# will-rowe/groot

Hardware: AMD Instinct MI355X
Metric: Mreads/s aligned (higher is better)
Workload: dtype u64

## Files before the change

### groot_amd/csrc/hip/align.hip

```cpp
#include <hip/hip_runtime.h>

#include "kernels_align.hpp"
#include "kernels_lean.hpp"
#include "launch.hpp"

namespace groot {

void launch_align(uint32_t pw, const AlignArgs &a, dim3 grid, hipStream_t st)
{
    const size_t lds = a.lds_stride_dw ? (size_t)kBlock * a.lds_stride_dw * 4 + 16 : 0;
    if (pw == 3) {
        if (lds) hipLaunchKernelGGL((align_kernel<3, true>), grid, dim3(kBlock), lds, st, a);
        else hipLaunchKernelGGL((align_kernel<3, false>), grid, dim3(kBlock), 0, st, a);
    } else if (pw == 11) {
        if (lds) hipLaunchKernelGGL((align_kernel<11, true>), grid, dim3(kBlock), lds, st, a);
        else hipLaunchKernelGGL((align_kernel<11, false>), grid, dim3(kBlock), 0, st, a);
    }
}

void launch_align_lean(uint32_t pw, const LeanArgs &a, dim3 grid, hipStream_t st)
{
    if (pw != 3) return;
    const size_t lds = (size_t)kBlock * a.lds_stride_dw * 4;
    if (a.max_len <= 128) hipLaunchKernelGGL((align_lean_kernel<3, 4>), grid, dim3(kBlock), lds, st, a);
    else if (a.max_len <= 160) hipLaunchKernelGGL((align_lean_kernel<3, 5>), grid, dim3(kBlock), lds, st, a);
    else hipLaunchKernelGGL((align_lean_kernel<3, 8>), grid, dim3(kBlock), lds, st, a);
}

void launch_align_path(uint32_t pw, const LeanArgs &a, dim3 grid, hipStream_t st)
{
    if (pw != 3) return;
// ... 8 lines not shown
```

### groot_amd/csrc/hip/ctx.hpp

```cpp
#pragma once

#include <hip/hip_runtime.h>

#include <algorithm>
#include <array>
#include <atomic>
#include <cstdlib>
#include <deque>
#include <map>
#include <memory>
#include <string>
#include <thread>
#include <vector>

#include "device_types.hpp"

using namespace groot;


template <class T> struct DevBuf {
    T *p = nullptr;
    size_t n = 0;
    hipError_t alloc(size_t count)
    {
// ... 24 lines not shown
    hipError_t reserve(size_t count) { return count <= n && p ? hipSuccess : alloc(count); }
    void release()
    {
        if (p) (void)hipHostFree(p);
        p = nullptr;
        n = 0;
    }
    ~PinBuf() { release(); }
};

struct Knobs {
    bool no_outcome_table = false, no_text_table = false, no_sig = false, force_rccl = false, small_buffers = false, open_stats = false, poison = false, lean = false, no_path = false,
         shared_slow = false, serial_tail = false, assign_global = false;
    uint32_t ec_slots = 0;
    uint32_t acov_slots = 0;
    static Knobs read()
    {
        Knobs k;
        k.no_outcome_table = getenv("GROOT_NO_OUTCOME_TABLE") != nullptr; k.no_text_table = getenv("GROOT_NO_TEXT_TABLE") != nullptr;
        k.no_sig = getenv("GROOT_NO_SIG") != nullptr;                     k.force_rccl = getenv("GROOT_FORCE_RCCL") != nullptr;
        k.small_buffers = getenv("GROOT_TEST_SMALL_BUFFERS") != nullptr;  k.open_stats = getenv("GROOT_OPEN_STATS") != nullptr;
        k.poison = getenv("GROOT_TEST_POISON") != nullptr;
        k.lean = getenv("GROOT_LEAN") != nullptr;
        k.no_path = getenv("GROOT_NO_PATH_PASS") != nullptr;
        k.shared_slow = getenv("GROOT_TEST_SHARED_SLOW") != nullptr;
        k.serial_tail = getenv("GROOT_SERIAL_TAIL") != nullptr;
        k.assign_global = getenv("GROOT_TEST_ASSIGN_GLOBAL") != nullptr;
        if (const char *e = getenv("GROOT_TEST_EC_SLOTS")) k.ec_slots = (uint32_t)std::min<unsigned long>(strtoul(e, nullptr, 10), 1ul << 30);
        if (const char *e = getenv("GROOT_TEST_ACOV_SLOTS")) k.acov_slots = (uint32_t)std::min<unsigned long>(strtoul(e, nullptr, 10), 1ul << 30);
        return k;
    }
};

namespace groot {
struct EcTable;
struct AcovTable;
}

struct EcBufs {
    uint32_t cap = 0;
    DevBuf<uint32_t> claim, graph;
    DevBuf<uint64_t> mask;
    DevBuf<unsigned long long> cnt;
    DevBuf<uint32_t> serial;
// ... 114 lines not shown
    hipEvent_t ev_seed = nullptr;
    hipEvent_t ev_walk = nullptr;
    hipEvent_t ev_h2d0 = nullptr, ev_h2d = nullptr, ev_compute = nullptr, ev_ctr = nullptr, ev_d2h0 = nullptr, ev_d2h = nullptr;
    hipEvent_t ev[14]{};
    groot_counts counts{};
    int status = GROOT_OK;
    std::string status_msg;
    groot_stage_ms ms{};
    SlotCounters ct;
    const uint8_t *seq() const { return input == IN_DEVICE ? ext_seq : d_seq.p; }
    const uint64_t *off() const { return input == IN_DEVICE ? ext_off : d_off.p; }
};

struct WorkSet {
    DevBuf<uint32_t> seed_count, seed_win, perm, perm_count, trav_cnt, tab_idx;
    DevBuf<uint32_t> perm2;
    DevBuf<uint4> packed;
    DevBuf<ReadRec> read_rec;
    DevBuf<uint4> vitem, split_list;
    DevBuf<uint32_t> vcount;
    DevBuf<groot_trav> trav_first;
    DevBuf<uint64_t> mask_first, sketches;
    DevBuf<groot_trav> ovf_trav;
    DevBuf<uint64_t> ovf_mask;
    DevBuf<uint32_t> ovf_cnt;
    hipEvent_t ev_free = nullptr;
    bool used = false;
    Slot *owner = nullptr;
    uint64_t ticket = 0;
};

// ... 131 lines not shown
```

### groot_amd/csrc/hip/device_types.hpp

```cpp
#pragma once

#include <cstdint>

#include <hip/hip_runtime.h>

#include "groot_hip.h"

namespace groot {

constexpr int kBlock = 256;
constexpr uint32_t kEmpty = 0xFFFFFFFFu;

enum : uint32_t {
    kFlagShortRead = 1u,
    kFlagLongRead = 2u,
    kFlagSeedOverflow = 4u,
    kFlagTravOverflow = 8u,
    kFlagOrdOverflow = 16u,
    kFlagOvfOverflow = 32u,
    kFlagQOverflow = 64u,
};

constexpr uint32_t kIncrCap = 8;
constexpr uint32_t kIncrCapBig = 2048;
constexpr uint32_t kSeedShards = 64, kSeedShardStride = 16;
constexpr uint32_t kOvfShards = 256;
// ... 182 lines not shown
    groot_trav *ovf_trav;
    uint64_t *ovf_mask;
    uint32_t *ovf_cnt;
    uint32_t ovf_cap;
    uint64_t *stk_hdr;
    uint64_t *stk_mask;
    uint32_t n_threads, stk_depth;
    uint32_t lds_stride_dw;
    uint32_t *incr_cnt, *incr_win;
    uint32_t incr_cap;
    uint32_t head_lanes;
    uint32_t round_lanes;
    const uint4 *vitem;
    const uint32_t *vcount;
    uint32_t vcap;
    const uint32_t *n_perm;
    const uint32_t *rest;
    uint32_t rest_lo;
    uint32_t refill;
    DeviceCounters *ctr;
};

struct alignas(16) LeanNode {
    uint32_t seq_off;
    uint32_t seq_len;
    uint32_t deg_kids;
    uint32_t pad;
    uint32_t edges[4];
    uint64_t first32;
    uint64_t mask[3];
};
static_assert(sizeof(LeanNode) == 64, "lean node record is one 64-byte line");
constexpr uint32_t kLeanNo = 0x80000000u;
// ... 14 lines not shown
    const WinRec *win_rec;
    const uint32_t *q_row;
    const uint8_t *seq;
    const uint4 *packed;
    uint32_t packed_q;
    const uint32_t *perm;
    const ReadRec *read_rec;
    uint32_t n_reads, first_read_id, n_windows, k;
    uint32_t update_weights;
    uint32_t lds_stride_dw;
    uint32_t max_len;
    uint32_t *attempts;
    groot_trav *trav_first;
    uint64_t *mask_first;
    uint32_t *trav_cnt;
    uint32_t *left;
    uint32_t *left_cnt;
    uint4 *stk;
    groot_trav *ovf_trav;
    uint64_t *ovf_mask;
    uint32_t *ovf_cnt;
    uint32_t ovf_cap;
    DeviceCounters *ctr;
    const uint4 *path_node;
    const uint32_t *path_text;
    const uint32_t *path_tag;
    const uint32_t *path_nodes;
    const uint64_t *path_tab;
    uint4 *hold;
};

// ... 4 lines not shown
```

### groot_amd/csrc/hip/groot_hip.hip

```cpp
#include <cstring>

#include <hip/hip_runtime.h>
#include <rocprim/rocprim.hpp>

#include <dlfcn.h>

#include <algorithm>
#include <cmath>
#include <cstdarg>
#include <cstdio>
#include <atomic>
#include <chrono>
#include <deque>
#include <iterator>
#include <array>
#include <map>
#include <tuple>
#include <memory>
#include <numeric>
#include <string>
#include <thread>
#include <vector>

#include "../common/cpus.hpp"
#include "../common/view_check.hpp"
#include "counters.hpp"
#include "ctx.hpp"
#include "kernels_misc.hpp"
#include "kernels_path.hpp"
#include "launch.hpp"

using namespace groot;

__attribute__((constructor)) static void groot_hw_queues() { setenv("GPU_MAX_HW_QUEUES", "8", 0); }

static thread_local std::string g_open_err;

static thread_local bool tl_background = false;

namespace groot {

int fail(groot_ctx *ctx, int code, const char *fmt, ...)
{
    char buf[1024];
    va_list ap;
// ... 434 lines not shown
    a.attempts = c->attempts_ptr;
    a.node_rec = c->node_rec.p;
    a.trav_first = w->trav_first.p;
    a.mask_first = w->mask_first.p;
    a.trav_cnt = w->trav_cnt.p;
    a.ovf_trav = w->ovf_trav.p;
    a.ovf_mask = w->ovf_mask.p;
    a.ovf_cnt = w->ovf_cnt.p;
    a.ovf_cap = c->ovf_cap;
    if (c->vcap) { a.vitem = w->vitem.p; a.vcount = w->vcount.p; a.vcap = c->vcap; }
    a.stk_hdr = c->stk_hdr.p;
    a.stk_mask = c->stk_mask.p;
    uint32_t blocks = std::min<uint32_t>((s->n_reads + kBlock - 1) / kBlock, c->align_threads / kBlock);
    if (c->dfs_frac < kSparseBelow && c->dfs_frac * (double)s->n_reads < 16.0 * (double)(blocks * (kBlock / 64))) blocks = std::max(1u, blocks / 2);
    else if (error_batch(c, s) && blocks >= 4) blocks /= 2;
    if ((s->lean_used || s->path_used) && c->lean_left_frac < 0.25) {
        uint32_t want = (uint32_t)(c->lean_left_frac * 1.25 * (double)s->n_reads / 64.0 / (kBlock / 64)) + 1u;
        blocks = std::max(1u, std::min(blocks, std::max(want, c->n_cu)));
    }
    a.n_threads = blocks * kBlock;
    a.stk_depth = c->stk_depth;
    {
        const uint32_t stride = (2 + 4 * ((s->max_len + 27) / 16)) | 1u;
        a.lds_stride_dw = (size_t)kBlock * stride * 4 <= 64 * 1024 ? stride : 0;
    }
    if (c->tab_capture) {
        a.incr_cnt = c->incr_cnt.p; a.incr_win = c->incr_win.p; a.incr_cap = c->incr_cap;
        HIP_TRY(c, hipMemsetAsync(c->incr_cnt.p, 0, (size_t)s->n_reads * sizeof(uint32_t), c->tstream));
    }
    a.head_lanes = s->mixed_len ? 16u : 0u;
#ifndef GROOT_REFILL_ERR
#define GROOT_REFILL_ERR 48
#endif
#ifndef GROOT_REFILL_MIXED
#define GROOT_REFILL_MIXED 2
#endif
    a.refill = s->mixed_len ? (uint32_t)GROOT_REFILL_MIXED : (error_batch(c, s) ? (uint32_t)GROOT_REFILL_ERR : 64u);
#ifdef GROOT_WORK_COUNTERS
    if (const char *e = getenv("GROOT_DEV_ROUND")) a.round_lanes = (uint32_t)atoi(e);
#endif
    a.ctr = s->d_ctr.p;
    const bool first_pass = s->lean_used || s->path_used;
    hipStream_t walk = first_pass ? c->astream : c->tstream;
    HIP_TRY(c, hipMemsetAsync(w->ovf_cnt.p, 0, (kOvfShards + 3) * sizeof(uint32_t), walk));
    const uint32_t lean_stride = lean_stride_dw(s->max_len);
    if (first_pass) {
        LeanArgs l{};
        l.nodes = c->lean_nodes.p; l.ext = c->lean_ext.p; l.bases2 = c->bases2.p; l.cn_pre2 = c->cn_pre2.p; l.win_ok = c->win_ok.p;
        l.win_rec = c->dix.win_rec; l.node_l2b = c->dix.node_l2b; l.q_row = c->q_row.p;
        l.seq = s->seq(); l.packed = s->packed_q ? w->packed.p : nullptr; l.packed_q = s->packed_q; l.perm = w->perm.p; l.read_rec = w->read_rec.p;
        l.n_reads = s->n_reads; l.first_read_id = s->first_read_id; l.n_windows = c->n_windows; l.k = c->k;
        l.update_weights = update_weights ? 1 : 0;
        l.lds_stride_dw = lean_stride; l.max_len = s->max_len;
        l.attempts = c->attempts_ptr;
        l.trav_first = w->trav_first.p; l.mask_first = w->mask_first.p; l.trav_cnt = w->trav_cnt.p;
        l.left = w->perm2.p; l.left_cnt = w->ovf_cnt.p + kOvfShards + 2; l.ctr = s->d_ctr.p;
        l.stk = c->lean_stk.p; l.ovf_trav = w->ovf_trav.p; l.ovf_mask = w->ovf_mask.p; l.ovf_cnt = w->ovf_cnt.p; l.ovf_cap = c->ovf_cap;
        const uint32_t lean_blocks = std::min<uint32_t>((s->n_reads + kBlock - 1) / kBlock, (uint32_t)(c->dfs_frac * 1.05 * (double)s->n_reads / kBlock) + 64u);
        if (s->path_used) {
            l.path_node = c->path_node.p; l.path_text = c->path_text.p; l.path_tag = c->path_tag.p; l.path_nodes = c->path_nodes.p; l.path_tab = c->path_tab.p;
            l.hold = c->path_hold.p;
            launch_align_path(c->pw, l, dim3(lean_blocks), c->astream);
        } else launch_align_lean(c->pw, l, dim3(lean_blocks), c->astream);
        HIP_TRY(c, hipGetLastError());
        a.perm = w->perm2.p;
        a.n_perm = l.left_cnt;
        a.rest = w->perm.p;
        a.rest_lo = lean_blocks * (uint32_t)kBlock;
        if (c->profiling) HIP_TRY(c, hipEventRecord(s->ev[13], c->astream));
        if (c->tstream != c->astream) {
            HIP_TRY(c, hipEventRecord(s->ev_walk, c->astream));
            HIP_TRY(c, hipStreamWaitEvent(c->tstream, s->ev_walk, 0));
        }
    }
    launch_align(c->pw, a, dim3(blocks), c->tstream);
    HIP_TRY(c, hipGetLastError());
    return GROOT_OK;
}

static int launch_order_stage(groot_ctx *c, Slot *s, bool update_weights)
{
    WorkSet *w = &c->ws[s->set];
    const uint32_t n = s->n_reads;
// ... 47 lines not shown


static int run_batch_async(groot_ctx *c, Slot *s, bool update_weights)
{
    WorkSet *w = &c->ws[s->set];
    if (w->used) HIP_TRY(c, hipStreamWaitEvent(c->stream, w->ev_free, 0));
    HIP_TRY(c, hipMemsetAsync(s->d_ctr.p, 0, sizeof(DeviceCounters), c->stream));
    if (c->kn.poison) {
        const size_t n = s->n_reads;
        HIP_TRY(c, hipMemsetAsync(w->seed_count.p, 0, n * sizeof(uint32_t), c->stream));
        HIP_TRY(c, hipMemsetAsync(w->read_rec.p, 0, n * sizeof(ReadRec), c->stream));
        HIP_TRY(c, hipMemsetAsync(w->trav_cnt.p, 0, n * sizeof(uint32_t), c->stream));
        HIP_TRY(c, hipMemsetAsync(c->sort_key.p, 0xFF, n * sizeof(uint32_t), c->stream));
        if (w->tab_idx.p) HIP_TRY(c, hipMemsetAsync(w->tab_idx.p, 0xFF, n * sizeof(uint32_t), c->stream));
        HIP_TRY(c, hipMemsetAsync(c->todo_list.p, 0, n * sizeof(uint32_t), c->stream));
    }
    if (c->profiling) HIP_TRY(c, hipEventRecord(s->ev[1], c->stream));
    if (int rc = launch_seed_stage(c, s, update_weights)) return rc;
    if (c->profiling) HIP_TRY(c, hipEventRecord(s->ev[3], c->stream));
    HIP_TRY(c, hipEventRecord(s->ev_seed, c->stream));
    s->lean_used = c->lean && !c->tab_capture && s->n_reads && s->max_len <= kLeanMaxLen && c->dfs_frac >= 0.02;
    s->path_used = c->path && !c->tab_capture && s->n_reads && s->max_len <= kLeanMaxLen && c->dfs_frac >= 0.02;
    hipStream_t start = s->lean_used || s->path_used ? c->astream : c->tstream;
    HIP_TRY(c, hipStreamWaitEvent(start, s->ev_seed, 0));
    if (c->profiling) HIP_TRY(c, hipEventRecord(s->ev[11], start));
    if (int rc = launch_align_stage(c, s, update_weights)) return rc;
    if (c->profiling) HIP_TRY(c, hipEventRecord(s->ev[4], c->tstream));
    if (int rc = launch_order_stage(c, s, update_weights)) return rc;
    if (c->profiling) HIP_TRY(c, hipEventRecord(s->ev[5], c->tstream));
    HIP_TRY(c, hipEventRecord(w->ev_free, c->tstream));
// ... 432 lines not shown
}

}

extern "C" {

void groot_params_default(groot_params *p)
{
    if (!p) return;
    memset(p, 0, sizeof *p);
    p->containment_threshold = 0.99;
    p->max_read_len = 256;
    p->max_batch_reads = 1u << 20;
    p->max_seeds_per_read = 8;
    p->pipeline_depth = 3;
}

int groot_hip_device_count(int *n)
{
    if (!n) return GROOT_E_INVALID;
    int c = 0;
    hipError_t e = hipGetDeviceCount(&c);
    if (e != hipSuccess) {
        *n = 0;
        return fail(nullptr, GROOT_E_DEVICE, "hipGetDeviceCount: %s", hipGetErrorString(e));
    }
    *n = c;
    return GROOT_OK;
}

// ... 1069 lines not shown
    HIP_TRY(c, c->long_count.alloc(4));
    HIP_TRY(c, hipMemset(c->long_count.p, 0, 4 * sizeof(uint32_t)));
    {
        std::vector<uint32_t> iota(R);
        std::iota(iota.begin(), iota.end(), 0u);
        HIP_TRY(c, upload(c->perm_in, iota.data(), iota.size()));
    }
    if (int rc = alloc_seed_slots(c, c->prm.max_seeds_per_read)) return rc;
    c->vcap = c->kn.small_buffers ? 8u : std::max<uint32_t>(4096, R / 4);
    for (WorkSet &w : c->ws) {
        HIP_TRY(c, w.seed_count.alloc(R));
        HIP_TRY(c, w.read_rec.alloc(R));
        HIP_TRY(c, w.perm.alloc(R));
        HIP_TRY(c, w.perm_count.alloc(4));
        if (c->lean || c->path) {
            HIP_TRY(c, w.perm2.alloc(R));
            HIP_TRY(c, w.packed.alloc((size_t)R * (c->prm.max_read_len <= 128 ? 2 : 4)));
        }
        if (c->prm.keep_sketches) HIP_TRY(c, w.sketches.alloc((size_t)R * s));
        HIP_TRY(c, w.trav_first.alloc((size_t)R + c->vcap));
        HIP_TRY(c, w.mask_first.alloc(((size_t)R + c->vcap) * c->pw));
        HIP_TRY(c, w.trav_cnt.alloc((size_t)R + c->vcap));
        HIP_TRY(c, w.vitem.alloc(std::max<uint32_t>(c->vcap, 1)));
        HIP_TRY(c, w.split_list.alloc(kLongListCap));
        HIP_TRY(c, w.vcount.alloc(4));
        HIP_TRY(c, hipMemset(w.vcount.p, 0, 4 * sizeof(uint32_t)));
    }
    HIP_TRY(c, c->trav_off.alloc(R));
    if (c->lean || c->path) HIP_TRY(c, c->lean_stk.alloc((size_t)R * 4));
    if (c->path) HIP_TRY(c, c->path_hold.alloc((size_t)R * 3 * kPathHold));
    for (WorkSet &w : c->ws) HIP_TRY(c, w.ovf_cnt.alloc(kOvfShards + 3));
// ... 828 lines not shown
```

### groot_amd/csrc/hip/kernels_align.hpp

```cpp
#pragma once

#include "kernels_common.hpp"

namespace groot {


enum : uint32_t { PH_FETCH, PH_SCAN, PH_DFS, PH_WAIT, PH_DONE, PH_FORK, PH_FORKWAIT, PH_JOIN };
#ifndef GROOT_FORK_MIN
#define GROOT_FORK_MIN 3
#endif
constexpr uint32_t kForkMin = GROOT_FORK_MIN;
constexpr uint32_t kClsHelper = 0x1000u;
constexpr uint32_t kCoopMin = 6;
constexpr uint32_t kCoopWant = 0xFFFFFFFEu;
#ifndef GROOT_COOP_MAX_ASK
#define GROOT_COOP_MAX_ASK 8
#endif
constexpr uint32_t kCoopMaxAsk = GROOT_COOP_MAX_ASK;
#ifndef GROOT_TL_LATE_US
#define GROOT_TL_LATE_US 3000
#endif
#ifndef GROOT_WAVE_CHUNK
#define GROOT_WAVE_CHUNK 128
#endif
constexpr uint32_t kWaveChunk = GROOT_WAVE_CHUNK;

__device__ __forceinline__ uint64_t match_or_n(uint64_t x, unsigned c)
{
    return ~(nonzero_bytes(x ^ (kOnes * c)) & nonzero_bytes(x ^ (kOnes * 'N'))) & kHi1;
}
__device__ __forceinline__ uint64_t low_bytes(int n) { return n <= 0 ? 0 : (n >= 8 ? kHi1 : (kHi1 >> (8 * (8 - n)))); }

template <int PW> struct RecRegs {
    static constexpr int NQ = (int)(sizeof(NodeRec<PW>) / 16);
    uint32_t d[NQ * 4];
    __device__ __forceinline__ void load(const NodeRec<PW> *rp)
    {
        const uint4 *q = reinterpret_cast<const uint4 *>(rp);
#pragma unroll
        for (int i = 0; i < NQ; i++) {
            const uint4 v = q[i];
            d[4 * i] = v.x; d[4 * i + 1] = v.y; d[4 * i + 2] = v.z; d[4 * i + 3] = v.w;
        }
#pragma unroll
        for (int i = 0; i < NQ * 4; i++) asm volatile("" : "+v"(d[i]));
    }
// ... 26 lines not shown
#endif
    unsigned long long alns = 0, mapped = 0, multimapped = 0, panics = 0;
#ifdef GROOT_WORK_COUNTERS
    uint32_t ev = 0;
    uint32_t wc_iter = 0, wc_round0 = 0;
    unsigned long long wc_t[3] = {0, 0, 0};
    uint32_t wc_n[3] = {0, 0, 0};
    uint32_t wc_n0[3] = {0, 0, 0};
#define GROOT_EV(i) (ev |= 1u << (i))
#else
#define GROOT_EV(i) ((void)0)
#endif

    uint32_t phase = PH_WAIT;
    const uint32_t nv = a.vitem ? min((uint32_t)__builtin_amdgcn_readfirstlane((int)*a.vcount), a.vcap) : 0u;
    const uint32_t n_seeded = min(a.n_reads, (uint32_t)__builtin_amdgcn_readfirstlane((int)a.ctr->seeded_reads));
    const uint32_t n_list = a.n_perm ? min(a.n_reads, (uint32_t)__builtin_amdgcn_readfirstlane((int)*a.n_perm)) : n_seeded;
    const uint32_t n_rest = a.rest && n_seeded > a.rest_lo ? n_seeded - a.rest_lo : 0u;
    const uint32_t n_todo = nv + (a.perm ? min(a.n_reads, n_list + n_rest) : a.n_reads);
#ifndef GROOT_MIXED_ROUND_LANES
#define GROOT_MIXED_ROUND_LANES 32
#endif
    uint32_t U = a.head_lanes ? (uint32_t)GROOT_MIXED_ROUND_LANES : 64u;
    if (a.round_lanes) U = a.round_lanes;
    else
        while (U > 1u && n_todo < U * (gridDim.x * (uint32_t)(kBlock / 64))) U >>= 1;
    const uint32_t n_rounds = (n_todo + U - 1u) / U;
    const uint32_t head_rounds = (n_rounds >> 3) | 1u;
    const uint32_t Uh = a.head_lanes ? min(a.head_lanes, U) : U;
    const uint32_t head_slots = min(head_rounds * U, n_todo);
    const uint32_t head_small = (head_slots + Uh - 1u) / Uh;
    uint32_t chunk_len = 0, chunk_base = 0;
    bool head_done = head_small == 0;
    const uint32_t chunk_rounds = a.head_lanes ? 1u : kWaveChunk / 64u;
    auto take_chunk = [&]() {
        uint32_t c = 0, tail = 0;
        if ((threadIdx.x & 63) == 0) {
            if (!head_done) c = atomicAdd(a.ovf_cnt + kOvfShards, 1u);
            if (head_done || c >= head_small) {
                tail = 1;
                c = atomicAdd(a.ovf_cnt + kOvfShards + 1, chunk_rounds);
            }
        }
        c = (uint32_t)__builtin_amdgcn_readfirstlane((int)c);
        tail = (uint32_t)__builtin_amdgcn_readfirstlane((int)tail);
        if (tail) {
            head_done = true;
            const unsigned long long b = (unsigned long long)head_slots + (unsigned long long)c * U;
            chunk_base = b > 0xFFFFFFFFull ? 0xFFFFFFFFu : (uint32_t)b;
            chunk_len = chunk_rounds * U;
        } else {
            chunk_base = c * Uh;
            chunk_len = min(Uh, head_slots - chunk_base);
        }
    };
    take_chunk();
#if defined(GROOT_WORK_COUNTERS) && GROOT_WORK_COUNTERS == 3
    const unsigned long long tl_start = wall_clock64();
    unsigned long long tl_round = tl_start, tl_coop = 0, tl_fork = 0, tl_read0 = 0;
    uint32_t tl_it0 = 0, tl_st0 = 0;
    uint32_t tl_rounds = 0, tl_ncoop = 0;
#endif
    uint32_t chunk_pos = 0;
    uint32_t slot = 0, r = 0;
    bool have_read = false;
    const uint8_t *p = nullptr;
    uint32_t len = 0, cnt = 0, qrow = 0, n_graphs = 0, ord = 0, read_id = 0;
    uint32_t sd0 = kEmpty, sd1 = kEmpty, sd2 = kEmpty, sd3 = kEmpty;
    uint32_t high_byte = 0;
    uint32_t cls = 0;
    long long last = -1;
    uint32_t done_graph = kEmpty, cur_graph = kEmpty;
    bool group_rc_called = false;
    uint32_t w = 0, g = 0, seed = 0, seed_s0 = 0, seed_len = 0, off0 = 0, l1_hi = 0, cn_cur = 0, cn_begin = 0, cn_end = 0;
    uint32_t rc = 0, level = 1;
    uint32_t sc_node = 0, sc_s0 = 0, sc_len = 0, sc_pos = 0, sc_end = 0;
    auto clip_lo = [&]() -> uint32_t { return level == 3u ? 1u : 0u; };
    auto eff = [&]() -> uint32_t { return len - (level >= 3u ? 1u : 0u); };
// ... 198 lines not shown
            const unsigned long long below = bhit ? bm & ((1ull << (__ffsll(bhit) - 1)) - 1ull) : bm;
            if (below & ~bdone) continue;
            const uint32_t w_top = below ? __shfl(w, 63 - __builtin_clzll(below)) + 1u : 0u;
            if (mine) { phase = (fk >> 8) & 7u; cls = 0; have_read = false; fk = 0; }
            if ((int)(threadIdx.x & 63u) == L) { fk = w_top; phase = PH_FETCH; }
        }
        }
#if defined(GROOT_WORK_COUNTERS) && GROOT_WORK_COUNTERS == 3
        tl_fork += wall_clock64() - tl_c1;
#endif
        const unsigned long long bf = __ballot(phase == PH_FETCH), bs = __ballot(phase == PH_SCAN), bd = __ballot(phase == PH_DFS);
        {
            const unsigned long long bw = __ballot(phase == PH_WAIT);
            const int cw = __popcll(bw);
            const uint32_t Uc = max(1u, min(chunk_len, min(U, 64u)));
            if (cw >= (int)((64u - Uc) + max(1u, a.refill * Uc / 64u)) || (cw && !(bf | bs | bd))) {
#if defined(GROOT_WORK_COUNTERS) && GROOT_WORK_COUNTERS == 1
                if ((threadIdx.x & 63) == 0 && wc_iter > 1) atomicAdd(&a.ctr->dbg[128 + min(63u, (wc_iter - wc_round0) / 2)], 1ull);
                if ((threadIdx.x & 63) == 0) atomicMax(&a.ctr->dbg[63], (unsigned long long)(wc_iter - wc_round0));
                wc_round0 = wc_iter;
#elif defined(GROOT_WORK_COUNTERS)
                wc_round0 = wc_iter;
#endif
#if defined(GROOT_WORK_COUNTERS) && GROOT_WORK_COUNTERS == 3
                if (chunk_base < n_todo) { tl_round = wall_clock64(); tl_rounds++; }
#endif
                const uint64_t base = chunk_base;
                if (base >= n_todo) {
                    if (phase == PH_WAIT) phase = PH_DONE;
                } else {
                    const uint32_t room = chunk_len - chunk_pos;
                    if (phase == PH_WAIT) {
                        const uint32_t rank = __builtin_amdgcn_mbcnt_hi((uint32_t)(bw >> 32), __builtin_amdgcn_mbcnt_lo((uint32_t)bw, 0u));
                        const uint64_t sl = base + chunk_pos + rank;
                        if (rank < room) {
                            if (sl < n_todo) { slot = (uint32_t)sl; phase = PH_FETCH; GROOT_EV(20); }
                            else phase = PH_DONE;
                        }
                    }
                    chunk_pos += min((uint32_t)cw, room);
                    if (chunk_pos >= chunk_len) { chunk_pos = 0; take_chunk(); }
                }
                continue;
            }
            if (!(bf | bs | bd)) break;
        }
        const int cf = __popcll(bf), cs = __popcll(bs), cd = __popcll(bd);
        const uint32_t run = (cd >= cs && cd >= cf) ? PH_DFS : (cs >= cf ? PH_SCAN : PH_FETCH);
        if (phase != run) continue;
        GROOT_EV(run);
#ifdef GROOT_WORK_COUNTERS
        const unsigned long long wc_t0 = wall_clock64();
        const uint32_t wc_steps0 = wc_iter;
#endif
        bool advance = false;

// ... 8 lines not shown
                GROOT_EV(3);
#if defined(GROOT_WORK_COUNTERS) && GROOT_WORK_COUNTERS == 2
                wc_n0[0] = wc_n[0]; wc_n0[1] = wc_n[1]; wc_n0[2] = wc_n[2];
#endif
#if defined(GROOT_WORK_COUNTERS) && GROOT_WORK_COUNTERS == 3
                tl_read0 = wall_clock64(); tl_it0 = wc_iter; tl_st0 = wc_n[0] + wc_n[1] + wc_n[2];
#endif
                const bool virt = slot < nv;
                uint32_t vlo = 0, vhi = 0;
                if (virt) {
                    const uint4 vi = a.vitem[slot];
                    r = vi.x; vlo = vi.y; vhi = vi.z;
                    if (r == kEmpty) { phase = PH_WAIT; continue; }
                } else {
                    const uint32_t so = slot - nv;
                    r = !a.perm ? so : so < n_list ? a.perm[so] : a.rest[a.rest_lo + (so - n_list)];
                }
                uint4 ra, rb;
                load32(a.read_rec + r, ra, rb);
                const uint32_t sc = ra.w;
                cnt = min(sc & (kRecSplit - 1u), a.seed_slots);
                cls = a.perm ? (sc >> 24) & 0x3Fu : 0x80u;
                if (sc & kRecAscending) cls |= 0x100u;
                if (sc & kRecSplit) cls |= 0xA00u;
                if (virt) { cnt = min(vhi, a.seed_slots); cls = 0x80u | 0x100u | 0x200u | 0x400u; }
                if (cnt == 0) { a.trav_cnt[r] = 0; phase = PH_WAIT; continue; }
                high_byte = sc >> 31;
                len = ra.z & ~kRecPacked;
                p = a.seq + ((uint64_t)ra.x | ((uint64_t)ra.y << 32));
                sd0 = rb.x; sd1 = rb.y; sd2 = rb.z; sd3 = rb.w;
                if (cls & 0x200u) sd0 = vlo;
// ... 420 lines not shown
    if ((threadIdx.x & 63) == 0)
        for (int i = 0; i < 3; i++) { atomicAdd(&a.ctr->dbg[24 + i], wc_t[i]); atomicAdd(&a.ctr->dbg[27 + i], (unsigned long long)wc_n[i]); }
#endif
    alns = block_sum(alns, red);
    mapped = block_sum(mapped, red);
    multimapped = block_sum(multimapped, red);
    panics = block_sum(panics, red);
    if (threadIdx.x == 0) {
        if (alns) atomicAdd(&a.ctr->alignments, alns);
        if (a.update_weights) {
            if (mapped) atomicAdd(&a.ctr->mapped, mapped);
            if (multimapped) atomicAdd(&a.ctr->multimapped, multimapped);
            if (panics) atomicAdd(&a.ctr->revcomp_panics, panics);
        }
    }
}


}
```

### groot_amd/csrc/hip/kernels_lean.hpp

```cpp
#pragma once

#include "kernels_common.hpp"
#include "kernels_path.hpp"

namespace groot {


#ifndef GROOT_LEAN_WAVES
#define GROOT_LEAN_WAVES 5
#endif
constexpr int kLeanWaves = GROOT_LEAN_WAVES;
#ifndef GROOT_LEAN_MAX_ITER
#define GROOT_LEAN_MAX_ITER 96
#endif
constexpr uint32_t kLeanMaxIter = GROOT_LEAN_MAX_ITER;

__device__ __forceinline__ uint64_t lean_lowmask(int n) { return n <= 0 ? 0ull : (n >= 32 ? ~0ull : ((1ull << (2 * n)) - 1ull)); }
__device__ __forceinline__ uint32_t lean_revcomp16(uint32_t v)
{
    uint32_t r = __brev(v);
    r = ((r & 0xAAAAAAAAu) >> 1) | ((r & 0x55555555u) << 1);
    return r ^ 0xAAAAAAAAu;
}
__device__ __forceinline__ uint64_t lean_funnel(uint32_t x0, uint32_t x1, uint32_t x2, uint32_t sh)
// ... 455 lines not shown
        const unsigned long long b = __ballot(st == ST_DEFER && why == y);
        if (b && (threadIdx.x & 63) == 0) atomicAdd(&a.ctr->dbg[160 + y], (unsigned long long)__popcll(b));
    }
    { const unsigned long long b = __ballot(st == ST_DONE && !ord); if (b && (threadIdx.x & 63) == 0) atomicAdd(&a.ctr->dbg[160], (unsigned long long)__popcll(b)); }
    for (uint32_t y = 11; y <= 13; y++) {
        const unsigned long long b = __ballot(st == ST_DEFER && why == y);
        if (b && (threadIdx.x & 63) == 0) atomicAdd(&a.ctr->dbg[160 + y], (unsigned long long)__popcll(b));
    }
    if (PATH)
        for (int i = 0; i < 5; i++) if (stops[i]) atomicAdd(&a.ctr->dbg[176 + i], (unsigned long long)stops[i]);
#endif
    const bool fin = st == ST_DONE;
    {
        const bool left = st == ST_DEFER && slot < n_todo;
        const unsigned long long lb = __ballot(left);
        if (lb) {
            const unsigned lane_ = threadIdx.x & 63u;
            const int first = __ffsll(lb) - 1;
            uint32_t at = 0;
            if ((int)lane_ == first) at = atomicAdd(a.left_cnt, (uint32_t)__popcll(lb));
            at = __shfl(at, first);
            if (left) a.left[at + (uint32_t)__popcll(lb & ((1ull << lane_) - 1ull))] = r;
        }
    }
    unsigned long long n_alns = 0, mapped = 0, multimapped = 0;
    if (fin) {
        a.trav_cnt[r] = ord;
        if (PATH)
            for (uint32_t o = 1; o < ord; o++) {
                const uint4 h0 = hold[3 * (o - 1)], h1 = hold[3 * (o - 1) + 1], h2 = hold[3 * (o - 1) + 2];
                groot_trav t_;
                t_.read_id = a.first_read_id + r; t_.graph_id = h0.x; t_.node = h0.y; t_.offset = h0.z;
                t_.ord = (uint16_t)(h0.w & 0xFFFFu); t_.flags = (uint8_t)(h0.w >> 16); t_.reserved = 0;
                const uint32_t shard = blockIdx.x & (kOvfShards - 1);
                const uint32_t at = atomicAdd(&a.ovf_cnt[shard], 1u);
                if (at < a.ovf_cap) {
                    const size_t q = (size_t)shard * a.ovf_cap + at;
// ... 50 lines not shown
```

### include/groot_hip.h

```cpp
#ifndef GROOT_HIP_H
#define GROOT_HIP_H

#include <stddef.h>
#include <stdint.h>

#include "groot_host.h"
#include "groot_index.h"

#ifdef __cplusplus
extern "C" {
#endif

typedef struct groot_ctx groot_ctx;

typedef struct groot_params {
    double   containment_threshold;
    uint32_t no_exact_align;
    uint32_t max_read_len;
    uint32_t max_batch_reads;
    uint32_t max_seeds_per_read;
    uint64_t max_batch_bases;
    uint32_t keep_sketches;
    uint32_t pipeline_depth;
    uint32_t results_on_device;
// ... 28 lines not shown
    float h2d, sketch_seed, align, sort, total, schedule, d2h, unpack;
    float first_seed_kernel, order_kernel;
    float list_pass, wall;
    float lean_pass;
} groot_stage_ms;

int groot_hip_device_count(int *n);
const char *groot_hip_last_error(const groot_ctx *ctx);

int groot_hip_open(groot_ctx **out, int device_id, const groot_index_view *idx, const groot_params *p);
#define GROOT_OPEN_BACKGROUND 1u
int groot_hip_open_flags(groot_ctx **out, int device_id, const groot_index_view *idx, const groot_params *p, uint32_t flags);
int groot_hip_open_wait(groot_ctx *ctx);
int groot_hip_open_abandon(groot_ctx *ctx);
void groot_hip_close(groot_ctx *ctx);

typedef struct groot_open_stats {
    double open_ms;
    double memo_ms;
    uint64_t memo_strings;
    uint64_t memo_tabulated;
    uint64_t memo_entries;
    uint64_t text_entries;
    uint64_t memo_hbm_bytes;
} groot_open_stats;
int groot_hip_open_stats(const groot_ctx *ctx, groot_open_stats *out);

int groot_hip_set_stream(groot_ctx *ctx, void *hip_stream);
int groot_hip_stream_join(groot_ctx *ctx, void *hip_stream);
int groot_hip_redo_status(groot_ctx *ctx, const uint32_t **d_status, uint32_t *redo_mask);
// ... 109 lines not shown
```

Before: 2370.

## Replace deferred-read list with per-wave bitmask and claim words in second pass

The lean/path first pass now writes a 64-bit ballot mask per wave of deferred reads instead of atomically compacting read ids into a list. The second-pass align kernel claims chunks of mask words, prefix-sums popcounts across the wave into LDS, and maps lanes to reads via nth-set-bit. It also adds top-up refills and moves block sizing into a helper with env overrides. This removes the compaction atomics and the indirect list loads, but adds LDS usage, wave-level scans and bit searches, and can leave lanes idle when masks are sparse.

```diff
diff --git a/groot_amd/csrc/hip/align.hip b/groot_amd/csrc/hip/align.hip
--- a/groot_amd/csrc/hip/align.hip
+++ b/groot_amd/csrc/hip/align.hip
@@ -8,13 +8,14 @@
 
 void launch_align(uint32_t pw, const AlignArgs &a, dim3 grid, hipStream_t st)
 {
+    const size_t claim = a.left_bits ? kClaimLdsBytes : 0;
     const size_t lds = a.lds_stride_dw ? (size_t)kBlock * a.lds_stride_dw * 4 + 16 : 0;
     if (pw == 3) {
-        if (lds) hipLaunchKernelGGL((align_kernel<3, true>), grid, dim3(kBlock), lds, st, a);
-        else hipLaunchKernelGGL((align_kernel<3, false>), grid, dim3(kBlock), 0, st, a);
+        if (lds) hipLaunchKernelGGL((align_kernel<3, true>), grid, dim3(kBlock), lds + claim, st, a);
+        else hipLaunchKernelGGL((align_kernel<3, false>), grid, dim3(kBlock), claim, st, a);
     } else if (pw == 11) {
-        if (lds) hipLaunchKernelGGL((align_kernel<11, true>), grid, dim3(kBlock), lds, st, a);
-        else hipLaunchKernelGGL((align_kernel<11, false>), grid, dim3(kBlock), 0, st, a);
+        if (lds) hipLaunchKernelGGL((align_kernel<11, true>), grid, dim3(kBlock), lds + claim, st, a);
+        else hipLaunchKernelGGL((align_kernel<11, false>), grid, dim3(kBlock), claim, st, a);
     }
 }
 
diff --git a/groot_amd/csrc/hip/ctx.hpp b/groot_amd/csrc/hip/ctx.hpp
--- a/groot_amd/csrc/hip/ctx.hpp
+++ b/groot_amd/csrc/hip/ctx.hpp
@@ -62,6 +62,8 @@
          shared_slow = false, serial_tail = false, assign_global = false;
     uint32_t ec_slots = 0;
     uint32_t acov_slots = 0;
+    uint32_t claim_words = 0;
+    uint32_t align_blocks = 0;
     static Knobs read()
     {
         Knobs k;
@@ -76,6 +78,8 @@
         k.assign_global = getenv("GROOT_TEST_ASSIGN_GLOBAL") != nullptr;
         if (const char *e = getenv("GROOT_TEST_EC_SLOTS")) k.ec_slots = (uint32_t)std::min<unsigned long>(strtoul(e, nullptr, 10), 1ul << 30);
         if (const char *e = getenv("GROOT_TEST_ACOV_SLOTS")) k.acov_slots = (uint32_t)std::min<unsigned long>(strtoul(e, nullptr, 10), 1ul << 30);
+        if (const char *e = getenv("GROOT_TEST_CLAIM_WORDS")) k.claim_words = (uint32_t)std::min<unsigned long>(strtoul(e, nullptr, 10), 64ul);
+        if (const char *e = getenv("GROOT_TEST_ALIGN_BLOCKS")) k.align_blocks = (uint32_t)std::min<unsigned long>(strtoul(e, nullptr, 10), 1ul << 16);
         return k;
     }
 };
@@ -220,7 +224,7 @@
 
 struct WorkSet {
     DevBuf<uint32_t> seed_count, seed_win, perm, perm_count, trav_cnt, tab_idx;
-    DevBuf<uint32_t> perm2;
+    DevBuf<uint64_t> left_bits;
     DevBuf<uint4> packed;
     DevBuf<ReadRec> read_rec;
     DevBuf<uint4> vitem, split_list;
diff --git a/groot_amd/csrc/hip/device_types.hpp b/groot_amd/csrc/hip/device_types.hpp
--- a/groot_amd/csrc/hip/device_types.hpp
+++ b/groot_amd/csrc/hip/device_types.hpp
@@ -10,6 +10,7 @@
 
 constexpr int kBlock = 256;
 constexpr uint32_t kEmpty = 0xFFFFFFFFu;
+constexpr uint32_t kClaimLdsBytes = (kBlock / 64) * 64 * (sizeof(uint64_t) + sizeof(uint32_t));
 
 enum : uint32_t {
     kFlagShortRead = 1u,
@@ -222,9 +223,11 @@
     const uint4 *vitem;
     const uint32_t *vcount;
     uint32_t vcap;
-    const uint32_t *n_perm;
-    const uint32_t *rest;
+    const uint64_t *left_bits;
+    const uint32_t *n_left;
     uint32_t rest_lo;
+    uint32_t claim_words;
+    uint32_t claim_fixed;
     uint32_t refill;
     DeviceCounters *ctr;
 };
@@ -269,7 +272,7 @@
     groot_trav *trav_first;
     uint64_t *mask_first;
     uint32_t *trav_cnt;
-    uint32_t *left;
+    uint64_t *left_bits;
     uint32_t *left_cnt;
     uint4 *stk;
     groot_trav *ovf_trav;
diff --git a/groot_amd/csrc/hip/groot_hip.hip b/groot_amd/csrc/hip/groot_hip.hip
--- a/groot_amd/csrc/hip/groot_hip.hip
+++ b/groot_amd/csrc/hip/groot_hip.hip
@@ -29,6 +29,7 @@
 #include "kernels_misc.hpp"
 #include "kernels_path.hpp"
 #include "launch.hpp"
+#include "second_pass.hpp"
 
 using namespace groot;
 
@@ -493,15 +494,23 @@
     uint32_t blocks = std::min<uint32_t>((s->n_reads + kBlock - 1) / kBlock, c->align_threads / kBlock);
     if (c->dfs_frac < kSparseBelow && c->dfs_frac * (double)s->n_reads < 16.0 * (double)(blocks * (kBlock / 64))) blocks = std::max(1u, blocks / 2);
     else if (error_batch(c, s) && blocks >= 4) blocks /= 2;
-    if ((s->lean_used || s->path_used) && c->lean_left_frac < 0.25) {
-        uint32_t want = (uint32_t)(c->lean_left_frac * 1.25 * (double)s->n_reads / 64.0 / (kBlock / 64)) + 1u;
-        blocks = std::max(1u, std::min(blocks, std::max(want, c->n_cu)));
-    }
+#ifndef GROOT_PASS2_CAP_CLEAN
+#define GROOT_PASS2_CAP_CLEAN 0
+#endif
+#ifndef GROOT_PASS2_CAP_ERR
+#define GROOT_PASS2_CAP_ERR 0
+#endif
+#ifndef GROOT_PASS2_CAP_MIXED
+#define GROOT_PASS2_CAP_MIXED 0
+#endif
+    const bool first_pass = s->lean_used || s->path_used;
+    const uint32_t pass2_cap = s->mixed_len ? (uint32_t)GROOT_PASS2_CAP_MIXED : error_batch(c, s) ? (uint32_t)GROOT_PASS2_CAP_ERR : (uint32_t)GROOT_PASS2_CAP_CLEAN;
+    blocks = second_pass_blocks(blocks, first_pass, c->lean_left_frac, s->n_reads, c->n_cu, pass2_cap, c->kn.align_blocks, kBlock / 64);
     a.n_threads = blocks * kBlock;
     a.stk_depth = c->stk_depth;
     {
         const uint32_t stride = (2 + 4 * ((s->max_len + 27) / 16)) | 1u;
-        a.lds_stride_dw = (size_t)kBlock * stride * 4 <= 64 * 1024 ? stride : 0;
+        a.lds_stride_dw = (size_t)kBlock * stride * 4 + (first_pass ? kClaimLdsBytes + 64 : 0) <= 64 * 1024 ? stride : 0;
     }
     if (c->tab_capture) {
         a.incr_cnt = c->incr_cnt.p; a.incr_win = c->incr_win.p; a.incr_cap = c->incr_cap;
@@ -515,11 +524,14 @@
 #define GROOT_REFILL_MIXED 2
 #endif
     a.refill = s->mixed_len ? (uint32_t)GROOT_REFILL_MIXED : (error_batch(c, s) ? (uint32_t)GROOT_REFILL_ERR : 64u);
+#ifndef GROOT_REFILL_PASS2
+#define GROOT_REFILL_PASS2 64
+#endif
+    if (first_pass && !s->mixed_len && !error_batch(c, s)) a.refill = (uint32_t)GROOT_REFILL_PASS2;
 #ifdef GROOT_WORK_COUNTERS
     if (const char *e = getenv("GROOT_DEV_ROUND")) a.round_lanes = (uint32_t)atoi(e);
 #endif
     a.ctr = s->d_ctr.p;
-    const bool first_pass = s->lean_used || s->path_used;
     hipStream_t walk = first_pass ? c->astream : c->tstream;
     HIP_TRY(c, hipMemsetAsync(w->ovf_cnt.p, 0, (kOvfShards + 3) * sizeof(uint32_t), walk));
     const uint32_t lean_stride = lean_stride_dw(s->max_len);
@@ -533,7 +545,7 @@
         l.lds_stride_dw = lean_stride; l.max_len = s->max_len;
         l.attempts = c->attempts_ptr;
         l.trav_first = w->trav_first.p; l.mask_first = w->mask_first.p; l.trav_cnt = w->trav_cnt.p;
-        l.left = w->perm2.p; l.left_cnt = w->ovf_cnt.p + kOvfShards + 2; l.ctr = s->d_ctr.p;
+        l.left_bits = w->left_bits.p; l.left_cnt = w->ovf_cnt.p + kOvfShards + 2; l.ctr = s->d_ctr.p;
         l.stk = c->lean_stk.p; l.ovf_trav = w->ovf_trav.p; l.ovf_mask = w->ovf_mask.p; l.ovf_cnt = w->ovf_cnt.p; l.ovf_cap = c->ovf_cap;
         const uint32_t lean_blocks = std::min<uint32_t>((s->n_reads + kBlock - 1) / kBlock, (uint32_t)(c->dfs_frac * 1.05 * (double)s->n_reads / kBlock) + 64u);
         if (s->path_used) {
@@ -542,10 +554,11 @@
             launch_align_path(c->pw, l, dim3(lean_blocks), c->astream);
         } else launch_align_lean(c->pw, l, dim3(lean_blocks), c->astream);
         HIP_TRY(c, hipGetLastError());
-        a.perm = w->perm2.p;
-        a.n_perm = l.left_cnt;
-        a.rest = w->perm.p;
+        a.left_bits = w->left_bits.p;
+        a.n_left = l.left_cnt;
         a.rest_lo = lean_blocks * (uint32_t)kBlock;
+        a.claim_words = second_pass_claim_words(c->lean_left_frac, s->mixed_len ? 32u : 64u, c->kn.claim_words);
+        a.claim_fixed = c->kn.claim_words ? 1u : 0u;
         if (c->profiling) HIP_TRY(c, hipEventRecord(s->ev[13], c->astream));
         if (c->tstream != c->astream) {
             HIP_TRY(c, hipEventRecord(s->ev_walk, c->astream));
@@ -623,6 +636,7 @@
         HIP_TRY(c, hipMemsetAsync(c->sort_key.p, 0xFF, n * sizeof(uint32_t), c->stream));
         if (w->tab_idx.p) HIP_TRY(c, hipMemsetAsync(w->tab_idx.p, 0xFF, n * sizeof(uint32_t), c->stream));
         HIP_TRY(c, hipMemsetAsync(c->todo_list.p, 0, n * sizeof(uint32_t), c->stream));
+        if (w->left_bits.p) HIP_TRY(c, hipMemsetAsync(w->left_bits.p, 0xFF, ((n + kBlock - 1) / kBlock) * (kBlock / 64) * sizeof(uint64_t), c->stream));
     }
     if (c->profiling) HIP_TRY(c, hipEventRecord(s->ev[1], c->stream));
     if (int rc = launch_seed_stage(c, s, update_weights)) return rc;
@@ -1085,6 +1099,13 @@
     p->max_batch_reads = 1u << 20;
     p->max_seeds_per_read = 8;
     p->pipeline_depth = 3;
+}
+
+void groot_hip_second_pass_plan(uint32_t blocks_in, double left_frac, uint32_t n_reads, uint32_t n_cu, uint32_t cap_per_cu, uint32_t forced_blocks,
+                                uint32_t round_reads, uint32_t forced_words, uint32_t *blocks, uint32_t *claim_words)
+{
+    if (blocks) *blocks = second_pass_blocks(blocks_in, true, left_frac, n_reads, n_cu, cap_per_cu, forced_blocks, kBlock / 64);
+    if (claim_words) *claim_words = second_pass_claim_words(left_frac, round_reads, forced_words);
 }
 
 int groot_hip_device_count(int *n)
@@ -2184,7 +2205,7 @@
         HIP_TRY(c, w.perm.alloc(R));
         HIP_TRY(c, w.perm_count.alloc(4));
         if (c->lean || c->path) {
-            HIP_TRY(c, w.perm2.alloc(R));
+            HIP_TRY(c, w.left_bits.alloc(((size_t)R + kBlock - 1) / kBlock * (kBlock / 64)));
             HIP_TRY(c, w.packed.alloc((size_t)R * (c->prm.max_read_len <= 128 ? 2 : 4)));
         }
         if (c->prm.keep_sketches) HIP_TRY(c, w.sketches.alloc((size_t)R * s));
diff --git a/groot_amd/csrc/hip/kernels_align.hpp b/groot_amd/csrc/hip/kernels_align.hpp
--- a/groot_amd/csrc/hip/kernels_align.hpp
+++ b/groot_amd/csrc/hip/kernels_align.hpp
@@ -30,6 +30,16 @@
     return ~(nonzero_bytes(x ^ (kOnes * c)) & nonzero_bytes(x ^ (kOnes * 'N'))) & kHi1;
 }
 __device__ __forceinline__ uint64_t low_bytes(int n) { return n <= 0 ? 0 : (n >= 8 ? kHi1 : (kHi1 >> (8 * (8 - n)))); }
+__device__ __forceinline__ uint32_t nth_set_bit(uint64_t x, uint32_t n)
+{
+    uint32_t pos = 0;
+#pragma unroll
+    for (uint32_t wd = 32; wd; wd >>= 1) {
+        const uint32_t c = (uint32_t)__popcll(x & ((1ull << wd) - 1ull));
+        if (n >= c) { n -= c; x >>= wd; pos += wd; }
+    }
+    return pos;
+}
 
 template <int PW> struct RecRegs {
     static constexpr int NQ = (int)(sizeof(NodeRec<PW>) / 16);
@@ -86,9 +96,10 @@
 
     uint32_t phase = PH_WAIT;
     const uint32_t nv = a.vitem ? min((uint32_t)__builtin_amdgcn_readfirstlane((int)*a.vcount), a.vcap) : 0u;
+#define behind_pass (a.left_bits != nullptr)
     const uint32_t n_seeded = min(a.n_reads, (uint32_t)__builtin_amdgcn_readfirstlane((int)a.ctr->seeded_reads));
-    const uint32_t n_list = a.n_perm ? min(a.n_reads, (uint32_t)__builtin_amdgcn_readfirstlane((int)*a.n_perm)) : n_seeded;
-    const uint32_t n_rest = a.rest && n_seeded > a.rest_lo ? n_seeded - a.rest_lo : 0u;
+    const uint32_t n_list = behind_pass ? min(a.n_reads, (uint32_t)__builtin_amdgcn_readfirstlane((int)*a.n_left)) : n_seeded;
+    const uint32_t n_rest = behind_pass && n_seeded > a.rest_lo ? n_seeded - a.rest_lo : 0u;
     const uint32_t n_todo = nv + (a.perm ? min(a.n_reads, n_list + n_rest) : a.n_reads);
 #ifndef GROOT_MIXED_ROUND_LANES
 #define GROOT_MIXED_ROUND_LANES 32
@@ -105,7 +116,53 @@
     uint32_t chunk_len = 0, chunk_base = 0;
     bool head_done = head_small == 0;
     const uint32_t chunk_rounds = a.head_lanes ? 1u : kWaveChunk / 64u;
+    auto chunk_words = [&]() -> bool { return behind_pass && chunk_base >= nv && chunk_base - nv < a.rest_lo; };
+    auto claim_lds = [&]() -> uint64_t * { return reinterpret_cast<uint64_t *>(lds_reads + (size_t)kBlock * a.lds_stride_dw) + (threadIdx.x & ~63u); };
+    auto claim_pre = [&]() -> uint32_t * {
+        return reinterpret_cast<uint32_t *>(reinterpret_cast<uint64_t *>(lds_reads + (size_t)kBlock * a.lds_stride_dw) + kBlock) + (threadIdx.x & ~63u);
+    };
+    auto take_claim = [&]() {
+        const uint32_t lane_ = threadIdx.x & 63u;
+        const uint32_t seeded = min(a.n_reads, (uint32_t)__builtin_amdgcn_readfirstlane((int)a.ctr->seeded_reads));
+        const uint32_t n_left = (uint32_t)__builtin_amdgcn_readfirstlane((int)*a.n_left);
+        const uint32_t lim_words = min(seeded, a.rest_lo);
+        const uint32_t n_words = (lim_words + 63u) >> 6;
+        const uint32_t rest = seeded > a.rest_lo ? seeded - a.rest_lo : 0u;
+        const uint32_t Wc = a.claim_fixed ? a.claim_words : min(64u, max(max(1u, a.claim_words * U / 64u), n_words / (8u * gridDim.x * (uint32_t)(kBlock / 64))));
+        const uint32_t cl_items = (nv + Uh - 1u) / Uh, cl_words = n_left ? (n_words + Wc - 1u) / Wc : 0u, cl_rest = (rest + U - 1u) / U;
+        for (;;) {
+            uint32_t c = 0;
+            if (lane_ == 0) c = atomicAdd(a.ovf_cnt + kOvfShards, 1u);
+            c = (uint32_t)__builtin_amdgcn_readfirstlane((int)c);
+            if (c < cl_items) { chunk_base = c * Uh; chunk_len = min(Uh, nv - chunk_base); return; }
+            c -= cl_items;
+            if (c < cl_words) {
+                const uint32_t w0 = c * Wc, wi = w0 + lane_;
+                uint64_t x = lane_ < Wc && wi < n_words ? a.left_bits[wi] : 0ull;
+                if (x && lim_words - wi * 64u < 64u) x &= (1ull << (lim_words - wi * 64u)) - 1ull;
+                uint32_t inc = (uint32_t)__popcll(x);
+#pragma unroll
+                for (uint32_t d = 1; d < 64u; d <<= 1) {
+                    const uint32_t t = __shfl_up(inc, d);
+                    if (lane_ >= d) inc += t;
+                }
+                const uint32_t total = (uint32_t)__builtin_amdgcn_readlane((int)inc, 63);
+                if (!total) continue;
+                __builtin_amdgcn_fence(__ATOMIC_ACQ_REL, "wavefront");
+                claim_lds()[lane_] = x; claim_pre()[lane_] = inc;
+                __builtin_amdgcn_fence(__ATOMIC_ACQ_REL, "wavefront");
+                __builtin_amdgcn_wave_barrier();
+                chunk_base = nv + w0 * 64u; chunk_len = total;
+                return;
+            }
+            c -= cl_words;
+            if (c < cl_rest) { chunk_base = nv + a.rest_lo + c * U; chunk_len = min(U, rest - c * U); return; }
+            chunk_base = 0xFFFFFFFFu; chunk_len = 0;
+            return;
+        }
+    };
     auto take_chunk = [&]() {
+        if (behind_pass) { take_claim(); return; }
         uint32_t c = 0, tail = 0;
         if ((threadIdx.x & 63) == 0) {
             if (!head_done) c = atomicAdd(a.ovf_cnt + kOvfShards, 1u);
@@ -134,6 +191,7 @@
     uint32_t tl_rounds = 0, tl_ncoop = 0;
 #endif
     uint32_t chunk_pos = 0;
+    bool topup = false;
     uint32_t slot = 0, r = 0;
     bool have_read = false;
     const uint8_t *p = nullptr;
@@ -362,7 +420,7 @@
             const unsigned long long bw = __ballot(phase == PH_WAIT);
             const int cw = __popcll(bw);
             const uint32_t Uc = max(1u, min(chunk_len, min(U, 64u)));
-            if (cw >= (int)((64u - Uc) + max(1u, a.refill * Uc / 64u)) || (cw && !(bf | bs | bd))) {
+            if (cw >= (int)((64u - Uc) + max(1u, a.refill * Uc / 64u)) || (cw && !(bf | bs | bd)) || topup) {
 #if defined(GROOT_WORK_COUNTERS) && GROOT_WORK_COUNTERS == 1
                 if ((threadIdx.x & 63) == 0 && wc_iter > 1) atomicAdd(&a.ctr->dbg[128 + min(63u, (wc_iter - wc_round0) / 2)], 1ull);
                 if ((threadIdx.x & 63) == 0) atomicMax(&a.ctr->dbg[63], (unsigned long long)(wc_iter - wc_round0));
@@ -371,23 +429,42 @@
                 wc_round0 = wc_iter;
 #endif
 #if defined(GROOT_WORK_COUNTERS) && GROOT_WORK_COUNTERS == 3
-                if (chunk_base < n_todo) { tl_round = wall_clock64(); tl_rounds++; }
-#endif
-                const uint64_t base = chunk_base;
-                if (base >= n_todo) {
+                if (chunk_base < (behind_pass ? 0xFFFFFFFFu : n_todo)) { tl_round = wall_clock64(); tl_rounds++; }
+#endif
+                const uint32_t n_end = behind_pass ? 0xFFFFFFFFu : n_todo;
+                const bool was_topup = topup;
+                topup = false;
+                if (chunk_base >= n_end) {
                     if (phase == PH_WAIT) phase = PH_DONE;
                 } else {
-                    const uint32_t room = chunk_len - chunk_pos;
+                    const uint64_t base = chunk_base;
+                    uint32_t room = chunk_len - chunk_pos;
+                    if (was_topup) room = min(room, U + (uint32_t)cw > 64u ? U + (uint32_t)cw - 64u : 0u);
                     if (phase == PH_WAIT) {
                         const uint32_t rank = __builtin_amdgcn_mbcnt_hi((uint32_t)(bw >> 32), __builtin_amdgcn_mbcnt_lo((uint32_t)bw, 0u));
-                        const uint64_t sl = base + chunk_pos + rank;
                         if (rank < room) {
-                            if (sl < n_todo) { slot = (uint32_t)sl; phase = PH_FETCH; GROOT_EV(20); }
+                            const uint32_t k = chunk_pos + rank;
+                            uint64_t sl = base + k;
+                            if (chunk_words()) {
+                                const uint32_t *pre = claim_pre();
+                                uint32_t j = 0;
+#pragma unroll
+                                for (uint32_t st = 32; st; st >>= 1)
+                                    if (pre[j + st - 1u] <= k) j += st;
+                                sl = base + 64u * j + nth_set_bit(claim_lds()[j], k - (j ? pre[j - 1u] : 0u));
+                            }
+                            if (sl < n_end) { slot = (uint32_t)sl; phase = PH_FETCH; GROOT_EV(20); }
                             else phase = PH_DONE;
                         }
                     }
-                    chunk_pos += min((uint32_t)cw, room);
-                    if (chunk_pos >= chunk_len) { chunk_pos = 0; take_chunk(); }
+                    const uint32_t took = min((uint32_t)cw, room);
+                    chunk_pos += took;
+                    if (chunk_pos >= chunk_len) {
+                        chunk_pos = 0;
+                        if (behind_pass) { __builtin_amdgcn_fence(__ATOMIC_ACQ_REL, "wavefront"); __builtin_amdgcn_wave_barrier(); }
+                        take_chunk();
+                        topup = behind_pass && took && took < (uint32_t)cw && chunk_base < n_end;
+                    }
                 }
                 continue;
             }
@@ -426,7 +503,7 @@
                     if (r == kEmpty) { phase = PH_WAIT; continue; }
                 } else {
                     const uint32_t so = slot - nv;
-                    r = !a.perm ? so : so < n_list ? a.perm[so] : a.rest[a.rest_lo + (so - n_list)];
+                    r = !a.perm ? so : a.perm[so];
                 }
                 uint4 ra, rb;
                 load32(a.read_rec + r, ra, rb);
@@ -877,6 +954,7 @@
             if (panics) atomicAdd(&a.ctr->revcomp_panics, panics);
         }
     }
+#undef behind_pass
 }
 
 
diff --git a/groot_amd/csrc/hip/kernels_lean.hpp b/groot_amd/csrc/hip/kernels_lean.hpp
--- a/groot_amd/csrc/hip/kernels_lean.hpp
+++ b/groot_amd/csrc/hip/kernels_lean.hpp
@@ -493,13 +493,9 @@
     {
         const bool left = st == ST_DEFER && slot < n_todo;
         const unsigned long long lb = __ballot(left);
-        if (lb) {
-            const unsigned lane_ = threadIdx.x & 63u;
-            const int first = __ffsll(lb) - 1;
-            uint32_t at = 0;
-            if ((int)lane_ == first) at = atomicAdd(a.left_cnt, (uint32_t)__popcll(lb));
-            at = __shfl(at, first);
-            if (left) a.left[at + (uint32_t)__popcll(lb & ((1ull << lane_) - 1ull))] = r;
+        if ((threadIdx.x & 63u) == 0u) {
+            a.left_bits[slot >> 6] = lb;
+            if (lb) atomicAdd(a.left_cnt, (uint32_t)__popcll(lb));
         }
     }
     unsigned long long n_alns = 0, mapped = 0, multimapped = 0;
diff --git a/groot_amd/csrc/hip/second_pass.hpp b/groot_amd/csrc/hip/second_pass.hpp
--- /dev/null
+++ b/groot_amd/csrc/hip/second_pass.hpp
@@ -0,0 +1,30 @@
+#pragma once
+
+#include <algorithm>
+#include <cstdint>
+
+namespace groot {
+
+constexpr double kSecondPassSparse = 0.25;
+
+inline uint32_t second_pass_claim_words(double left_frac, uint32_t round_reads, uint32_t forced)
+{
+    if (forced) return std::min(forced, 64u);
+    if (!(left_frac > 0.0)) return 64u;
+    const double w = (double)round_reads / (64.0 * left_frac);
+    return w >= 64.0 ? 64u : std::max(1u, (uint32_t)(w + 0.5));
+}
+
+inline uint32_t second_pass_blocks(uint32_t blocks, bool first_pass, double left_frac, uint32_t n_reads, uint32_t n_cu, uint32_t cap_per_cu, uint32_t forced,
+                                   uint32_t waves_per_block)
+{
+    if (!first_pass) return blocks;
+    if (forced) return std::max(1u, forced);
+    if (!(left_frac < kSecondPassSparse)) return blocks;
+    const uint32_t want = (uint32_t)(left_frac * 1.25 * (double)n_reads / 64.0 / (double)waves_per_block) + 1u;
+    uint32_t b = std::max(want, n_cu);
+    if (cap_per_cu) b = std::min(b, cap_per_cu * n_cu);
+    return std::max(1u, std::min(blocks, b));
+}
+
+}
diff --git a/include/groot_hip.h b/include/groot_hip.h
--- a/include/groot_hip.h
+++ b/include/groot_hip.h
@@ -66,6 +66,8 @@
 int groot_hip_open_wait(groot_ctx *ctx);
 int groot_hip_open_abandon(groot_ctx *ctx);
 void groot_hip_close(groot_ctx *ctx);
+void groot_hip_second_pass_plan(uint32_t blocks_in, double left_frac, uint32_t n_reads, uint32_t n_cu, uint32_t cap_per_cu, uint32_t forced_blocks,
+                                uint32_t round_reads, uint32_t forced_words, uint32_t *blocks, uint32_t *claim_words);
 
 typedef struct groot_open_stats {
     double open_ms;
```

Result: slower. 1096 (-53.8%).
